# itsdfish/DifferentialEvolutionMCMC.jl

Measured on AMD Instinct MI355X. Metric: particle-updates/sec (proposal+loglike+accept) at D=32, N=1e5, higher is better.
Workload: dtype f64; 1 GPU; cfg3: MvNormal full-Sigma D=32, N=100000 obs, n_groups=256x1, Np=256, sampler defaults, schedule=two_colour, loglike=direct; particles_per_gpu=65536, parallelism=groups sharded x1, one all-gather per migration

## Files before the change

differentialevolutionmcmc.jl_amd/csrc/demc_hip.cpp:

```cpp
#include "../../include/demc.h"
#include "../../include/demc_summary.h"
#include "../../include/demc_quantile.h"

#include <hip/hip_runtime.h>
#include <hip/hip_ext.h>
#include <hip/hiprtc.h>
#include <rccl/rccl.h>

#include <algorithm>
#include <cmath>
#include <cstdio>
#include <cstdlib>
#include <cstring>
#include <exception>
#include <new>
#include <string>
#include <vector>

#define DEMC_K1_EXTERN
#include "demc_kernels.hpp"
#define DEMC_LONGROW_EXTERN
#include "demc_longrow.hpp"
#define DEMC_FROZEN_EXTERN
#include "demc_frozen.hpp"
// ... 315 lines not shown
}

#define DEMC_USER_KPARAMS                                                   \
    struct UserKParams {                                                    \
        int n_groups, Np, D, a_lo, n_act, n_chunks, nhyper, with_prior;     \
        long long N, P;                                                     \
        const double* prop;                                                 \
        double* partial;                                                    \
        const double* data;                                                 \
        const double* hyper;                                                \
        const long long* dims;                                              \
        const int* glist;                                                   \
        int ndims, pad;                                                     \
    };
DEMC_USER_KPARAMS
#define DEMC_STR_(...) #__VA_ARGS__
#define DEMC_STR(...) DEMC_STR_(__VA_ARGS__)
const char* kUserStruct = R"SRC(
#ifndef INFINITY
#define INFINITY __builtin_huge_val()
#endif
#ifndef NAN
#define NAN __builtin_nan("")
#endif
)SRC" DEMC_STR(DEMC_USER_KPARAMS) "\n";
const char* kUserPrologue = R"SRC(
__device__ double demc_user_obs(const double* theta, int D, const double* data, long long N, long long i,
                                const double* hyper, int nhyper);
)SRC";
const char* kUserRowPrologue = R"SRC(
__device__ double demc_user_loglike_row(const double* theta, int D, const double* data, const long long* dims, int ndims,
                                        const double* hyper, int nhyper, int lane, int n_lanes);
#ifdef DEMC_USER_HAS_PRIOR
__device__ double demc_user_prior_row(const double* theta, int D, const double* hyper, int nhyper, int lane, int n_lanes);
#endif
)SRC";
const char* kUserRowKernel = R"SRC(
extern "C" __global__ __launch_bounds__(256) void k_user_row(UserKParams p) {
    __shared__ double s_part[4];
    const int q = blockIdx.x;
    const int g = q / p.n_act;
    const size_t slot = (size_t)(p.glist ? p.glist[g] : g) * p.Np + p.a_lo + (q - g * p.n_act);
    const double* th = p.prop + slot * p.D;
    double acc = demc_user_loglike_row(th, p.D, p.data, p.dims, p.ndims, p.hyper, p.nhyper, (int)threadIdx.x, 256);
#ifdef DEMC_USER_HAS_PRIOR
    if (p.with_prior) acc += demc_user_prior_row(th, p.D, p.hyper, p.nhyper, (int)threadIdx.x, 256);
#endif
    for (int o = 32; o > 0; o >>= 1) acc += __shfl_xor(acc, o);
    if ((threadIdx.x & 63) == 0) s_part[threadIdx.x >> 6] = acc;
    __syncthreads();
    if (threadIdx.x == 0) p.partial[slot] = (s_part[0] + s_part[1]) + (s_part[2] + s_part[3]);
}
)SRC";
const char* kUserKernel = R"SRC(
extern "C" __global__ __launch_bounds__(256) void k_user_loglike(UserKParams p) {
    const int q = blockIdx.x * 256 + threadIdx.x;
    const int chunk = blockIdx.y;
    if (q >= p.n_groups * p.n_act) return;
    const int g = q / p.n_act;
    const size_t slot = (size_t)(p.glist ? p.glist[g] : g) * p.Np + p.a_lo + (q - g * p.n_act);
    const double* th = p.prop + slot * p.D;
    const long long per = (p.N + p.n_chunks - 1) / p.n_chunks;
    const long long i0 = chunk * per, i1 = (i0 + per < p.N) ? i0 + per : p.N;
    double acc = 0.0;
    for (long long i = i0; i < i1; ++i) acc += demc_user_obs(th, p.D, p.data, p.N, i, p.hyper, p.nhyper);
    p.partial[(size_t)chunk * p.P + slot] = acc;
}
)SRC";

int chunks_filling_rounds(long long blocks, long long cap, double resident_wgs) {
    long long best = 1;
    double best_fill = 0.0;
    for (long long nc = 1; nc <= cap; ++nc) {
        const double wgs = (double)blocks * (double)nc;
        const double fill = wgs / (std::ceil(wgs / resident_wgs) * resident_wgs);
        if (fill > best_fill + 1e-9 || (fill > best_fill - 1e-9 && wgs <= 4.0 * resident_wgs)) { best = nc; best_fill = fill; }
    }
    return (int)best;
}

int clock_buffer(demc_handle* h, size_t wgs, unsigned long long** out) {
    *out = nullptr;
    if (!h->timing) return DEMC_OK;
    if (wgs > h->clk_cap) {
        if (h->clk_dev) { HIPCHK(hipStreamSynchronize(h->stream)); hipFree(h->clk_dev); h->clk_dev = nullptr; h->clk_cap = 0; }
        ALLOC(h->clk_dev, 3 * wgs);
        h->clk_cap = wgs;
    }
    HIPCHK(hipMemsetAsync(h->clk_dev, 0, 3 * wgs * sizeof(unsigned long long), h->stream));
    h->clk_n = wgs;
    *out = h->clk_dev;
    return DEMC_OK;
}

const char* kSimKernelSource =
#include "demc_simlike_src.inc"
    ;

int launch_sim_loglike(demc_handle* h, KParams& k, long long n_prop) {
    SimKParams s;
    std::memset(&s, 0, sizeof s);
    s.n_groups = k.n_groups; s.Np = k.Np; s.D = k.D; s.a_lo = k.a_lo; s.n_act = k.n_act; s.group_offset = k.group_offset;
    s.n_sim = h->sim_n; s.nhyper = h->user_nhyper > 0 ? h->user_nhyper - 1 : 0;
    s.n_obs = h->N; s.iter = k.iter; s.seed = k.seed; s.sweep = k.sweep; s.entity_base = h->sim_entity_base;
    s.bandwidth = h->sim_bw; s.n_pow = std::pow((double)h->sim_n, -0.2);
    s.prop = k.prop; s.partial = k.partial; s.obs = h->data; s.hyper = h->user_hyper ? h->user_hyper + 1 : nullptr;
    s.logtab = h->sim_logtab; s.glist = k.glist; s.k_max = h->sim_kmax;
    const size_t lds = h->sim_est == EST_KDE_CHOICE ? sim_choice_lds(h->sim_n) : (size_t)h->sim_n * sizeof(double);
    h->last.k2 = demc_handle::K2_SIM; h->last.k2_key = InstKey{{h->sim_kind, h->sim_est}};
    if (h->sim_kind == SIM_USER) {
        size_t sz = sizeof s;
        void* cfg[] = {HIP_LAUNCH_PARAM_BUFFER_POINTER, &s, HIP_LAUNCH_PARAM_BUFFER_SIZE, &sz, HIP_LAUNCH_PARAM_END};
        tick(h, 2, true, true);
        const hipError_t e = hipModuleLaunchKernel(h->user_kernel, (unsigned)n_prop, 1, 1, 256, 1, 1, 0, h->stream, nullptr, cfg);
        tick(h, 2, false, true);
        if (e != hipSuccess) return fail(h, DEMC_EHIP, std::string("hipModuleLaunchKernel: ") + hipGetErrorString(e));
        return DEMC_OK;
    }
    const Inst<SimFn>* e = nullptr;
    PICK(e, "k_sim_loglike", kSim, h->sim_kind, h->sim_est);
    tick(h, 2, true);
    LAUNCH_T(h, e->fn, dim3((unsigned)n_prop), dim3(256), lds, s);
    tick(h, 2, false);
    return DEMC_OK;
}

int launch_ode_loglike(demc_handle* h, KParams& k) {
    OdeKParams o;
    std::memset(&o, 0, sizeof o);
    o.n_groups = k.n_groups; o.Np = k.Np; o.D = k.D; o.a_lo = k.a_lo; o.n_act = k.n_act;
    o.T = (int)h->N; o.substeps = h->ode_substeps;
    std::memcpy(o.u0, h->ode_u0, sizeof o.u0);
    o.h = h->ode_h; o.h2 = 0.5 * h->ode_h; o.h6 = h->ode_h / 6.0;
    o.prop = k.prop; o.partial = k.partial; o.obs = h->data; o.glist = k.glist;
    const Inst<OdeFn>* e = nullptr;
    PICK(e, "k_ode_loglike", kOde, ODE_LV);
    h->last.k2 = demc_handle::K2_ODE; h->last.k2_key = e->key;
    const size_t lds = (size_t)h->N * 2 * sizeof(double);
    tick(h, 2, true);
    LAUNCH_T(h, e->fn, dim3((unsigned)k.n_groups, (unsigned)((k.n_act + 255) / 256)), dim3(256), lds, o);
    tick(h, 2, false);
    return DEMC_OK;
}

int launch_loglike(demc_handle* h, KParams& k) {
    const long long n_prop = (long long)k.n_groups * k.n_act;
    if (n_prop == 0) return DEMC_OK;
    switch (h->family) {
        case FAM_MVN_FULL:
        case FAM_MVN_ISO: {
            const bool suff = h->c.loglike_mode == DEMC_LOGLIKE_SUFFSTAT;
            k.n_partials = 1;
            if (k.direct) {
                const long long blocks = (n_prop + 255) / 256;
                long long cap = h->N / 64;
                if (cap > h->partial_cap) cap = h->partial_cap;
                if (cap < 1) cap = 1;
                const Inst<ChunkFn>* e = nullptr;
                PICK(e, "k_direct_mvn", kDirect, h->dp_direct);
                if (int rc = wgs_per_cu(h, (const void*)e->fn, &h->direct_wgs_per_cu)) return rc;
                const int n_chunks = chunks_filling_rounds(blocks, cap, (double)h->direct_wgs_per_cu * h->n_cus);
                h->last.k2 = demc_handle::K2_DIRECT_MVN; h->last.k2_key = e->key;
                unsigned long long* clk = nullptr;
                if (int rc = clock_buffer(h, (size_t)blocks * (size_t)n_chunks, &clk)) return rc;
                tick(h, 2, true);
                LAUNCH_T(h, e->fn, dim3((unsigned)blocks, (unsigned)n_chunks), dim3(256), 0, k, n_chunks, clk);
                tick(h, 2, false);
                k.n_partials = n_chunks;
            } else if (!suff) {
                const Inst<CrossFn>* e = nullptr;
                PICK(e, "k_cross_mfma", kCross, h->ks_t <= 1 ? 1 : h->ks_t <= 2 ? 2 : h->ks_t <= 4 ? 4 : h->ks_t <= 8 ? 8 : 16, 4);
                h->last.k2 = demc_handle::K2_CROSS_MFMA; h->last.k2_key = e->key;
                tick(h, 2, true);
                const long long n_ptiles = (n_prop + 255) / 256;
                int n_chunks = 8;
                while (n_ptiles * n_chunks < 1024 && n_chunks * 2 <= 32 && h->n_tiles / (n_chunks * 2) >= 16) n_chunks *= 2;
                if (h->n_tiles < n_chunks) n_chunks = (int)(h->n_tiles > 0 ? h->n_tiles : 1);
                const int n_kpass = h->n_kpass;
                if (n_chunks * n_kpass > h->partial_cap) n_chunks = h->partial_cap / n_kpass;
                if (n_chunks < 1) return fail(h, DEMC_EINVAL, "data dimension too large for the partial-sum workspace");
                const int grid2 = (int)(n_ptiles * n_chunks);
                for (int kp = 0; kp < n_kpass; ++kp) {
                    const int k0 = kp * 4 * h->ks_t, part0 = kp * n_chunks;
                    LAUNCH_T(h, e->fn, dim3(grid2), dim3(256), 0, k, h->Ypad, h->dpad, k0, h->Xf, h->n_tiles, n_chunks, part0);
                }
                tick(h, 2, false);
                k.n_partials = n_chunks * n_kpass;
            }
        } break;
        case FAM_GAUSSIAN:
        case FAM_BINOMIAL:
        case FAM_LBA:
        case FAM_LNR:
        case FAM_RASTRIGIN: {
            long long cap = h->N / 32;
            if (cap > h->partial_cap) cap = h->partial_cap;
            if (cap < 1 || h->family == FAM_RASTRIGIN) cap = 1;
            if (int rc = wgs_per_cu(h, (const void*)k_obs_loglike, &h->obs_wgs_per_cu)) return rc;
            int n_chunks = chunks_filling_rounds((n_prop + 255) / 256, cap, (double)h->obs_wgs_per_cu * h->n_cus);
            if (h->family == FAM_LBA) {
                const Inst<ChunkFn>*e = nullptr, *e3 = nullptr;
                PICK(e, "k_lba_wave", kLbaWave, h->n_acc == 3 ? 3 : h->n_acc == 2 ? 2 : 0);
                PICK(e3, "k_lba_wave", kLbaWave, 3);
                if (int rc = wgs_per_cu(h, (const void*)e3->fn, &h->lba_wave_wgs_per_cu)) return rc;
                long long capw = h->N / 1024;
                if (capw > h->partial_cap) capw = h->partial_cap;
                if (capw < 1) capw = 1;
                int nc = chunks_filling_rounds((n_prop + 3) / 4, capw, (double)h->lba_wave_wgs_per_cu * h->n_cus);
                h->last.k2 = demc_handle::K2_LBA_WAVE;
                unsigned long long* clk = nullptr;
                if (int rc = clock_buffer(h, (size_t)((n_prop + 3) / 4) * (size_t)nc, &clk)) return rc;
                tick(h, 2, true);
                LAUNCH_T(h, e->fn, dim3((unsigned)((n_prop + 3) / 4), (unsigned)nc), dim3(256), 0, k, nc, clk);
                tick(h, 2, false);
                k.n_partials = nc;
                break;
            }
            h->last.k2 = demc_handle::K2_OBS;
            tick(h, 2, true);
            LAUNCH_T(h, k_obs_loglike, dim3((unsigned)((n_prop + 255) / 256), (unsigned)n_chunks), dim3(256), 0,
                               k, n_chunks);
            tick(h, 2, false);
            k.n_partials = n_chunks;
        } break;
        case FAM_USER: {
            long long want = (262144 + n_prop - 1) / n_prop;
            long long cap = h->N / 32;
            if (cap < 1) cap = 1;
            if (want > cap) want = cap;
            if (want > h->partial_cap) want = h->partial_cap;
            if (h->user_row) want = 1;
            UserKParams u;
            u.n_groups = k.n_groups; u.Np = k.Np; u.D = k.D; u.a_lo = k.a_lo; u.n_act = k.n_act; u.n_chunks = (int)want;
            u.nhyper = h->user_nhyper; u.with_prior = h->c.fitness_kind == DEMC_FITNESS_POSTERIOR ? 1 : 0;
            u.N = h->N; u.P = h->P; u.prop = k.prop; u.partial = k.partial;
            u.data = h->data; u.hyper = h->user_hyper; u.dims = h->user_dims; u.glist = k.glist; u.ndims = h->user_ndims; u.pad = 0;
            size_t sz = sizeof u;
            void* cfg[] = {HIP_LAUNCH_PARAM_BUFFER_POINTER, &u, HIP_LAUNCH_PARAM_BUFFER_SIZE, &sz, HIP_LAUNCH_PARAM_END};
            h->last.k2 = h->user_row ? demc_handle::K2_USER_ROW : demc_handle::K2_USER;
            tick(h, 2, true, true);
            hipError_t e = h->user_row
                ? hipModuleLaunchKernel(h->user_kernel, (unsigned)n_prop, 1, 1, 256, 1, 1, 0, h->stream, nullptr, cfg)
                : hipModuleLaunchKernel(h->user_kernel, (unsigned)((n_prop + 255) / 256), (unsigned)want, 1, 256, 1, 1, 0,
                                        h->stream, nullptr, cfg);
            tick(h, 2, false, true);
            if (e != hipSuccess) return fail(h, DEMC_EHIP, std::string("hipModuleLaunchKernel: ") + hipGetErrorString(e));
            k.n_partials = (int)want;
        } break;
        case FAM_SIM: {
            if (int rc = launch_sim_loglike(h, k, n_prop)) return rc;
            k.n_partials = 1;
        } break;
        case FAM_ODE_LV: {
            if (int rc = launch_ode_loglike(h, k)) return rc;
            k.n_partials = 1;
        } break;
        case FAM_HIER_BINOMIAL:
        case FAM_HIER_GAUSSIAN: {
            h->last.k2 = demc_handle::K2_HIER;
            tick(h, 2, true);
            LAUNCH_T(h, k_hier_loglike, dim3((unsigned)n_prop), dim3(256), 0, k);
            tick(h, 2, false);
            k.n_partials = 1;
        } break;
        default:
            return fail(h, DEMC_EUNSUPPORTED, "model family not set or not registered");
    }
    return DEMC_OK;
}

bool is_mvn(int fam) { return fam == FAM_MVN_FULL || fam == FAM_MVN_ISO; }

void set_tail_flags(demc_handle* h, KParams& k) {
    const demc_config& c = h->c;
    const bool suff = c.loglike_mode == DEMC_LOGLIKE_SUFFSTAT;
    k.fuse_prep = is_mvn(h->family) ? 1 : 0;
    k.prep_mfma = (h->family == FAM_MVN_FULL && k.lpp >= 4 && k.lpp <= 16 && h->d <= 32) ? 1 : 0;
    k.sx = (k.fuse_prep && suff) ? h->sx : nullptr;
    k.Ainv = (h->family == FAM_MVN_FULL) ? h->Ainv : nullptr;
    const long long obs_work = (h->family == FAM_HIER_GAUSSIAN) ? h->N * (h->d > 0 ? h->d : 1) : h->N;
    const bool cheap_obs = ((h->family == FAM_GAUSSIAN || h->family == FAM_BINOMIAL || h->family == FAM_RASTRIGIN) &&
                            h->N / k.lpp <= 512) ||
                           (h->hier_scr && obs_work / k.lpp <= 4096);
    const bool hist_private = c.schedule == DEMC_SCHED_SYNCHRONOUS && c.partner_kind == DEMC_PARTNER_HISTORY && k.mode == MODE_STEP &&
                              !(c.proposal_kind == 0 && k.iter <= c.burnin);
    const bool phase_private = c.schedule == DEMC_SCHED_TWO_COLOUR || c.schedule == DEMC_SCHED_SEQUENTIAL || k.mode == MODE_IDENT || hist_private;
    h->tf_cheap_obs = cheap_obs;
    k.fuse_obs = (cheap_obs && phase_private && c.fuse != 1) ? 1 : 0;
    k.fuse_accept = (((k.fuse_prep && suff) || k.fuse_obs) && c.fuse != 1 && phase_private) ? 1 : 0;
    k.write_prop = (!k.fuse_accept || k.trace) ? 1 : 0;
}
int lean_level(const demc_handle* h, const KParams& k) {
    const demc_config& c = h->c;
    const bool base = k.mode == MODE_STEP && c.proposal_kind == 0 && c.partner_kind == DEMC_PARTNER_CURRENT && c.update_kind == 0 &&
                      c.fitness_kind == 0 && c.kappa == 1.0 && !k.trace && !h->rp_active;
    return !base ? 0 : (c.theta_snooker == 0.0 && c.n_blocks == 0) ? 1 : 2;
}
bool is_plain(const demc_handle* h, const KParams& k) { return lean_level(h, k) == 1; }
int lean_hist(const demc_handle* h, const KParams& k) {
    const demc_config& c = h->c;
    const bool base = k.mode == MODE_STEP && c.proposal_kind == 0 && c.partner_kind == DEMC_PARTNER_HISTORY && c.update_kind == 0 &&
                      c.fitness_kind == 0 && c.kappa == 1.0 && !k.trace && !h->rp_active;
    return !base ? 0 : (c.theta_snooker == 0.0 && c.n_blocks == 0) ? 1 : 2;
}
int tail_of(const KParams& k) { return k.prep_mfma ? TAIL_PREP_MFMA : k.fuse_prep ? TAIL_PREP : k.fuse_obs ? TAIL_OBS : TAIL_NONE; }

int launch_phase(demc_handle* h, KParams k) {
    const long long n_prop = (long long)k.n_groups * k.n_act;
    if (n_prop == 0) return DEMC_OK;
    const demc_config& c = h->c;
    set_tail_flags(h, k);
    const int wg = k.lpp > 256 ? 512 : 256;
// ... 2233 lines not shown
```

differentialevolutionmcmc.jl_amd/csrc/demc_instances.hpp:

```cpp
#pragma once
#include <cstddef>
#include <string>

namespace demc {

constexpr int kMaxKey = 7;
struct InstKey { int v[kMaxKey]; };
constexpr bool same_key(const InstKey& a, const InstKey& b) {
    for (int i = 0; i < kMaxKey; ++i)
        if (a.v[i] != b.v[i]) return false;
    return true;
}

template <typename Fn>
struct Inst {
    Fn fn;
    InstKey key;
    std::string (*name)(const InstKey&);
};

template <typename I, size_t N>
constexpr const I* find_inst(const I (&tab)[N], const InstKey& key) {
    for (const I& e : tab)
        if (same_key(e.key, key)) return &e;
    return nullptr;
}
template <typename I, size_t N>
constexpr bool unique_keys(const I (&tab)[N]) {
    for (size_t i = 0; i < N; ++i)
        for (size_t j = i + 1; j < N; ++j)
            if (same_key(tab[i].key, tab[j].key)) return false;
    return true;
}

inline std::string int_list(const InstKey& k, int n) {
    std::string s;
    for (int i = 0; i < n; ++i) s += (i ? "," : "") + std::to_string(k.v[i]);
    return s;
}
inline const char* tf(int v) { return v == 0 ? "false" : v == 1 ? "true" : "2"; }
inline std::string name_propose(const InstKey& k) {
    static const char* const tails[4] = {"TAIL_NONE", "TAIL_PREP", "TAIL_PREP_MFMA", "TAIL_OBS"};
    return "k_propose<" + std::to_string(k.v[0]) + "," + tf(k.v[1]) + "," + tails[k.v[2] & 3] + "," + tf(k.v[3]) + "," + tf(k.v[4]) +
           (k.v[5] ? ",true>" : ">");
}
inline std::string name_res_mvn(const InstKey& k) {
    return "k_res_mvn<" + std::to_string(k.v[0]) + "," + tf(k.v[1]) + "," + std::to_string(k.v[2]) +
           (k.v[3] ? "," + std::to_string(k.v[3]) : "") + (k.v[5] ? ",iso" : "") + (k.v[6] ? ",direct" : "") + ">";
}
inline std::string name_frozen(const InstKey& k) { return "k_frozen_sweep<" + std::to_string(k.v[0]) + (k.v[3] ? ",big>" : ">"); }
inline std::string name_longrow(const InstKey& k) { return "k_longrow<" + int_list(k, 1) + ">"; }
inline std::string name_res_obs(const InstKey& k) { return "k_res_obs<" + int_list(k, 1) + ">"; }
inline std::string name_cross(const InstKey& k) { return "k_cross_mfma<" + int_list(k, 2) + ">"; }
inline std::string name_direct(const InstKey& k) { return "k_direct_mvn<" + int_list(k, 1) + ">"; }
inline std::string name_lba_wave(const InstKey&) { return "k_lba_wave"; }
inline std::string name_sim(const InstKey& k) {
    return std::string("k_sim_loglike<") + (k.v[1] == EST_KDE ? "kde" : k.v[1] == EST_FREQ ? "frequency" : "kde_choice") + "," +
           (k.v[0] == SIM_NORMAL ? "normal" : k.v[0] == SIM_BINOMIAL ? "binomial" : k.v[0] == SIM_LNR ? "lnr" : "user") + ">";
}
inline std::string name_ode(const InstKey& k) { return std::string("k_ode_loglike<") + (k.v[0] == ODE_LV ? "lv" : "?") + ">"; }

using K1Fn = void (*)(KParams);
using K1Inst = Inst<K1Fn>;
using ChunkFn = void (*)(KParams, int, unsigned long long*);
using CrossFn = void (*)(KParams, const double*, int, int, const double*, int, int, int);
using SimFn = void (*)(SimKParams);
using OdeFn = void (*)(OdeKParams);
#define DEMC_ENTRY(KERNEL, NAME, ...) {KERNEL<__VA_ARGS__>, {{__VA_ARGS__}}, NAME},
#define DEMC_E_PROPOSE(...) DEMC_ENTRY(k_propose, name_propose, __VA_ARGS__)
#define DEMC_E_RES_MVN(...) DEMC_ENTRY(k_res_mvn, name_res_mvn, __VA_ARGS__)
#define DEMC_E_FROZEN(...) DEMC_ENTRY(k_frozen_sweep, name_frozen, __VA_ARGS__)
#define DEMC_E_LONGROW(...) DEMC_ENTRY(k_longrow, name_longrow, __VA_ARGS__)
#define DEMC_E_RES_OBS(...) DEMC_ENTRY(k_res_obs, name_res_obs, __VA_ARGS__)
#define DEMC_E_DIRECT(...) DEMC_ENTRY(k_direct_mvn, name_direct, __VA_ARGS__)
#define DEMC_E_CROSS(...) DEMC_ENTRY(k_cross_mfma, name_cross, __VA_ARGS__)
#define DEMC_E_LBA_WAVE(...) DEMC_ENTRY(k_lba_wave, name_lba_wave, __VA_ARGS__)
#define DEMC_E_SIM(...) DEMC_ENTRY(k_sim_loglike, name_sim, __VA_ARGS__)
#define DEMC_E_SIM_CHOICE(SIM) {k_sim_choice<SIM>, {{SIM, EST_KDE_CHOICE}}, name_sim},
#define DEMC_E_ODE(...) DEMC_ENTRY(k_ode_loglike, name_ode, __VA_ARGS__)
constexpr K1Inst kPropose[] = {DEMC_K1_PHASE_INSTANCES(DEMC_E_PROPOSE) DEMC_K1_RES_INSTANCES(DEMC_E_PROPOSE) DEMC_K1_STREAM_INSTANCES(DEMC_E_PROPOSE)};
constexpr K1Inst kResMvn[] = {DEMC_RESMVN_INSTANCES(DEMC_E_RES_MVN) DEMC_RESMVN_INSTANCES_DIR(DEMC_E_RES_MVN)};
constexpr K1Inst kFrozen[] = {DEMC_FROZEN_INSTANCES(DEMC_E_FROZEN)};
constexpr K1Inst kLongrow[] = {DEMC_LONGROW_INSTANCES(DEMC_E_LONGROW)};
constexpr K1Inst kResObs[] = {DEMC_RESOBS_INSTANCES(DEMC_E_RES_OBS)};
constexpr Inst<ChunkFn> kDirect[] = {DEMC_DIRECT_INSTANCES(DEMC_E_DIRECT)};
constexpr Inst<CrossFn> kCross[] = {DEMC_CROSS_INSTANCES(DEMC_E_CROSS)};
constexpr Inst<ChunkFn> kLbaWave[] = {DEMC_LBA_WAVE_INSTANCES(DEMC_E_LBA_WAVE)};
constexpr Inst<SimFn> kSim[] = {DEMC_SIM_INSTANCES(DEMC_E_SIM) DEMC_SIM_CHOICE_INSTANCES(DEMC_E_SIM_CHOICE)};
constexpr Inst<OdeFn> kOde[] = {DEMC_ODE_INSTANCES(DEMC_E_ODE)};
static_assert(unique_keys(kPropose) && unique_keys(kResMvn) && unique_keys(kFrozen) && unique_keys(kLongrow) && unique_keys(kResObs) &&
                  unique_keys(kCross) && unique_keys(kDirect) && unique_keys(kLbaWave) && unique_keys(kSim) && unique_keys(kOde),
              "an instance list names the same template arguments twice");

}
```

differentialevolutionmcmc.jl_amd/csrc/demc_kernels.hpp:

```cpp
#pragma once
#include <type_traits>
#include "demc_device.hpp"

namespace demc {

enum Family : int {
    FAM_GAUSSIAN = 0, FAM_MVN_ISO = 1, FAM_MVN_FULL = 2, FAM_BINOMIAL = 3, FAM_HIER_BINOMIAL = 4,
    FAM_HIER_GAUSSIAN = 5, FAM_LBA = 6, FAM_LNR = 7, FAM_RASTRIGIN = 8, FAM_USER = 100
};
enum Mode : int { MODE_STEP = 0, MODE_IDENT = 1 };

struct DimTab {
    double lo, hi;
    double a, b;
    double c;
    int kind, ref;
};

struct DimSeg {
    int start, pad;
    DimTab t;
    double pad2;
};
constexpr int kMaxDimSeg = 16;
// ... 1629 lines not shown
        }
        DEMC_STAMP(20);
    }
    if (RES) __syncthreads();
    DEMC_STAMP(10);
    }
}

#define DEMC_K1_PHASE_INSTANCES(X) \
    X(256, false, TAIL_NONE, false, 0, false) X(256, false, TAIL_PREP, false, 0, false) \
    X(256, false, TAIL_PREP_MFMA, false, 0, false) X(256, false, TAIL_OBS, false, 0, false) \
    X(256, true, TAIL_NONE, false, 0, false) X(256, true, TAIL_PREP, false, 0, false) \
    X(256, true, TAIL_PREP_MFMA, false, 0, false) X(256, true, TAIL_OBS, false, 0, false) \
    X(256, true, TAIL_NONE, false, 1, false) X(256, true, TAIL_PREP, false, 1, false) \
    X(256, true, TAIL_PREP_MFMA, false, 1, false) X(256, true, TAIL_OBS, false, 1, false) \
    X(512, false, TAIL_NONE, false, 0, false) X(512, false, TAIL_PREP, false, 0, false) \
    X(512, false, TAIL_PREP_MFMA, false, 0, false) X(512, false, TAIL_OBS, false, 0, false) \
    X(256, true, TAIL_NONE, false, 2, false) X(256, true, TAIL_PREP, false, 2, false) \
    X(256, true, TAIL_PREP_MFMA, false, 2, false) X(256, true, TAIL_OBS, false, 2, false) \
    X(256, false, TAIL_NONE, false, 1, false) X(256, false, TAIL_PREP, false, 1, false) \
    X(256, false, TAIL_PREP_MFMA, false, 1, false) X(256, false, TAIL_OBS, false, 1, false) \
    X(256, false, TAIL_NONE, false, 2, false) X(256, false, TAIL_PREP, false, 2, false) \
    X(256, false, TAIL_PREP_MFMA, false, 2, false) X(256, false, TAIL_OBS, false, 2, false)
#define DEMC_K1_RES_INSTANCES(X) \
    X(256, true, TAIL_NONE, true, 0, false) X(256, true, TAIL_PREP, true, 0, false) \
    X(256, true, TAIL_PREP_MFMA, true, 0, false) X(256, true, TAIL_OBS, true, 0, false) \
    X(512, true, TAIL_NONE, true, 0, false) X(512, true, TAIL_PREP, true, 0, false) \
    X(512, true, TAIL_PREP_MFMA, true, 0, false) X(512, true, TAIL_OBS, true, 0, false) \
    X(256, true, TAIL_NONE, true, 1, false) X(256, true, TAIL_PREP, true, 1, false) \
    X(256, true, TAIL_PREP_MFMA, true, 1, false) X(256, true, TAIL_OBS, true, 1, false) \
    X(512, true, TAIL_NONE, true, 1, false) X(512, true, TAIL_PREP, true, 1, false) \
    X(512, true, TAIL_PREP_MFMA, true, 1, false) X(512, true, TAIL_OBS, true, 1, false) \
    X(256, true, TAIL_NONE, true, 2, false) X(256, true, TAIL_PREP, true, 2, false) \
    X(256, true, TAIL_PREP_MFMA, true, 2, false) X(256, true, TAIL_OBS, true, 2, false) \
    X(512, true, TAIL_NONE, true, 2, false) X(512, true, TAIL_PREP, true, 2, false) \
    X(512, true, TAIL_PREP_MFMA, true, 2, false) X(512, true, TAIL_OBS, true, 2, false)
#define DEMC_K1_STREAM_INSTANCES(X) \
    X(256, true, TAIL_PREP, true, 0, true) X(256, true, TAIL_PREP_MFMA, true, 0, true) \
    X(256, true, TAIL_PREP, true, 1, true) X(256, true, TAIL_PREP_MFMA, true, 1, true) \
    X(256, true, TAIL_PREP, true, 2, true) X(256, true, TAIL_PREP_MFMA, true, 2, true) \
    X(512, true, TAIL_PREP, true, 0, true) X(512, true, TAIL_PREP_MFMA, true, 0, true) \
    X(512, true, TAIL_PREP, true, 1, true) X(512, true, TAIL_PREP_MFMA, true, 1, true) \
    X(512, true, TAIL_PREP, true, 2, true) X(512, true, TAIL_PREP_MFMA, true, 2, true)
#ifdef DEMC_K1_EXTERN
#define DEMC_X_(...) extern template __global__ void k_propose<__VA_ARGS__>(KParams);
DEMC_K1_PHASE_INSTANCES(DEMC_X_)
DEMC_K1_RES_INSTANCES(DEMC_X_)
DEMC_K1_STREAM_INSTANCES(DEMC_X_)
#undef DEMC_X_
#endif

template <int KS, int MT>
__global__ __launch_bounds__(256, 2) void k_cross_mfma(KParams p, const double* __restrict__ Ypad, int dpad, int k0,
                                                       const double* __restrict__ Xf, int n_tiles, int n_chunks,
                                                       int part0) {
    const int lane = threadIdx.x & 63, wave = threadIdx.x >> 6;
    const int chunk = blockIdx.x % n_chunks;
    const int ptile = blockIdx.x / n_chunks;
    const int n_prop = p.n_groups * p.n_act;
    const int q0 = (ptile * 4 + wave) * (MT * 16);
    const int ksx = dpad >> 2;

    double a[MT][KS];
#pragma unroll
    for (int mt = 0; mt < MT; ++mt) {
        const int q = q0 + mt * 16 + (lane & 15);
        const bool ok = q < n_prop;
        const size_t slot = ok ? (size_t)slot_of(p, q) : 0;
        const double* yrow = Ypad + slot * dpad + k0 + (lane >> 4);
#pragma unroll
        for (int ks = 0; ks < KS; ++ks) {
            const double v = yrow[4 * ks];
            a[mt][ks] = ok ? v : 0.0;
        }
    }
    d4 acc[MT];
#pragma unroll
    for (int mt = 0; mt < MT; ++mt) acc[mt] = (d4){0.0, 0.0, 0.0, 0.0};

    const int per = (n_tiles + n_chunks - 1) / n_chunks;
    const int t0 = chunk * per, t1 = (t0 + per < n_tiles) ? t0 + per : n_tiles;
    const size_t tstride = (size_t)ksx * 64;
    const double* xb = Xf + (size_t)(k0 >> 2) * 64 + lane;
    double b0[KS], b1[KS];
    {
        const double* x = xb + (size_t)(t0 < t1 ? t0 : n_tiles) * tstride;
#pragma unroll
        for (int ks = 0; ks < KS; ++ks) b0[ks] = x[ks * 64];
    }
    for (int t = t0; t < t1; t += 2) {
        {
            const double* x = xb + (size_t)(t + 1 < t1 ? t + 1 : n_tiles) * tstride;
#pragma unroll
            for (int ks = 0; ks < KS; ++ks) b1[ks] = x[ks * 64];
        }
#pragma unroll
        for (int ks = 0; ks < KS; ++ks)
#pragma unroll
            for (int mt = 0; mt < MT; ++mt)
                acc[mt] = __builtin_amdgcn_mfma_f64_16x16x4f64(a[mt][ks], b0[ks], acc[mt], 0, 0, 0);
        {
            const double* x = xb + (size_t)(t + 2 < t1 ? t + 2 : n_tiles) * tstride;
#pragma unroll
            for (int ks = 0; ks < KS; ++ks) b0[ks] = x[ks * 64];
        }
#pragma unroll
        for (int ks = 0; ks < KS; ++ks)
#pragma unroll
            for (int mt = 0; mt < MT; ++mt)
                acc[mt] = __builtin_amdgcn_mfma_f64_16x16x4f64(a[mt][ks], b1[ks], acc[mt], 0, 0, 0);
    }
#pragma unroll
    for (int mt = 0; mt < MT; ++mt)
#pragma unroll
        for (int r = 0; r < 4; ++r) {
            double v = acc[mt][r];
            v += __shfl_xor(v, 1);
            v += __shfl_xor(v, 2);
            v += __shfl_xor(v, 4);
            v += __shfl_xor(v, 8);
            const int q = q0 + mt * 16 + (lane >> 4) + 4 * r;
            if ((lane & 15) == 0 && q < n_prop) p.partial[(size_t)(part0 + chunk) * p.P + slot_of(p, q)] = v;
        }
}
#define DEMC_CROSS_INSTANCES(X) X(1, 4) X(2, 4) X(4, 4) X(8, 4) X(16, 4)

template <int DP>
__device__ __forceinline__ void direct_mvn_rows(const KParams& p, int pblock, int chunk, int n_chunks) {
    const int q = pblock * 256 + threadIdx.x;
    const bool ok = q < p.n_groups * p.n_act;
    const size_t slot = ok ? (size_t)slot_of(p, q) : 0;
    double m[DP];
    const double* mrow = p.Ypad + slot * p.dpad;
#pragma unroll
    for (int k = 0; k < DP; ++k) m[k] = (ok && k < p.d) ? mrow[k] : 0.0;
    const long long per = (p.N + n_chunks - 1) / n_chunks;
    const long long i0 = chunk * per, i1 = (i0 + per < p.N) ? i0 + per : p.N;
    double acc[4] = {0.0, 0.0, 0.0, 0.0};
    const double* z = p.data + i0 * DP;
    for (long long i = i0; i < i1; ++i, z += DP) {
#pragma unroll
        for (int k = 0; k < DP; k += 4) {
#pragma unroll
            for (int e = 0; e < 4; ++e) {
                const double r = z[k + e] - m[k + e];
                acc[e] = fma(r, r, acc[e]);
            }
        }
    }
    if (ok) p.partial[(size_t)chunk * p.P + slot] = (acc[0] + acc[1]) + (acc[2] + acc[3]);
}

typedef int zs16 __attribute__((ext_vector_type(16)));
typedef double zd8 __attribute__((ext_vector_type(8)));
__device__ __forceinline__ void zslice_ask(zs16& lo, zs16& hi, const double* row) {
    asm volatile("s_load_dwordx16 %0, %2, 0x0\n\ts_load_dwordx16 %1, %2, 0x40" : "=&s"(lo), "=&s"(hi) : "s"(row) : "memory");
    __builtin_amdgcn_sched_barrier(0);
}
__device__ __forceinline__ void zslice_wait(zs16& lo, zs16& hi) {
    asm volatile("s_waitcnt lgkmcnt(0)" : "+s"(lo), "+s"(hi));
    __builtin_amdgcn_sched_barrier(0);
}
__device__ __forceinline__ void zslice_fma(const zs16& lo, const zs16& hi, const double (&m0)[16], const double (&m1)[16],
                                           double (&a0)[2], double (&a1)[2]) {
    const zd8 zl = __builtin_bit_cast(zd8, lo), zh = __builtin_bit_cast(zd8, hi);
#pragma unroll
    for (int k = 0; k < 16; ++k) {
        const double z = k < 8 ? zl[k & 7] : zh[k & 7];
        const double r0 = z - m0[k], r1 = z - m1[k];
        a0[k & 1] = fma(r0, r0, a0[k & 1]);
        a1[k & 1] = fma(r1, r1, a1[k & 1]);
    }
}
__device__ __forceinline__ void direct_mvn_slices(const KParams& p, int pblock, int chunk, int n_chunks) {
    __shared__ double s_other[256];
    __shared__ int s_slot[256];
    constexpr int kNoSlot = -1;
    const int lane = threadIdx.x & 63, wave = __builtin_amdgcn_readfirstlane(threadIdx.x >> 6);
    const int s = wave >> 1, h = wave & 1;
    const int n_prop = p.n_groups * p.n_act;
    const int t0 = h * 128 + lane, t1 = t0 + 64;
    double m0[16], m1[16];
    {
        const bool ok0 = pblock * 256 + t0 < n_prop, ok1 = pblock * 256 + t1 < n_prop;
        const int slot0 = ok0 ? slot_of(p, pblock * 256 + t0) : 0, slot1 = ok1 ? slot_of(p, pblock * 256 + t1) : 0;
        if (s == 0) {
            s_slot[t0] = ok0 ? slot0 : kNoSlot;
            s_slot[t1] = ok1 ? slot1 : kNoSlot;
        }
        const double *mrow0 = p.Ypad + (size_t)slot0 * p.dpad + 16 * s, *mrow1 = p.Ypad + (size_t)slot1 * p.dpad + 16 * s;
#pragma unroll
        for (int k = 0; k < 16; ++k) {
            m0[k] = (ok0 && 16 * s + k < p.d) ? mrow0[k] : 0.0;
            m1[k] = (ok1 && 16 * s + k < p.d) ? mrow1[k] : 0.0;
        }
    }
    const long long per = (p.N + n_chunks - 1) / n_chunks;
    const long long i0 = chunk * per, i1 = (i0 + per < p.N) ? i0 + per : p.N;
    const int n = (int)(i1 - i0);
    double a0[2] = {0.0, 0.0}, a1[2] = {0.0, 0.0};
    if (n > 0) {
        const double* z = p.data + i0 * 32 + 16 * s;
        zs16 alo, ahi, blo, bhi;
        zslice_ask(alo, ahi, z);
        for (int left = n; left >= 2; left -= 2, z += 64) {
            zslice_wait(alo, ahi);
            zslice_ask(blo, bhi, z + 32);
            zslice_fma(alo, ahi, m0, m1, a0, a1);
            zslice_wait(blo, bhi);
            zslice_ask(alo, ahi, left > 2 ? z + 64 : z + 32);
            zslice_fma(blo, bhi, m0, m1, a0, a1);
        }
        zslice_wait(alo, ahi);
        if (n & 1) zslice_fma(alo, ahi, m0, m1, a0, a1);
    }
    const double sum0 = a0[0] + a0[1], sum1 = a1[0] + a1[1];
    if (s == 1) {
        s_other[t0] = sum0;
        s_other[t1] = sum1;
    }
    __syncthreads();
    if (s == 0) {
        double* part = p.partial + (size_t)chunk * p.P;
        const int slot0 = s_slot[t0], slot1 = s_slot[t1];
        if (slot0 != kNoSlot) part[slot0] = sum0 + s_other[t0];
        if (slot1 != kNoSlot) part[slot1] = sum1 + s_other[t1];
    }
}

template <int DP>
__global__ __launch_bounds__(256) void k_direct_mvn(KParams p, int n_chunks, unsigned long long* __restrict__ clk) {
    int pblock = blockIdx.x, chunk = blockIdx.y;
    if ((n_chunks & 7) == 0) {
        const unsigned lin = blockIdx.y * gridDim.x + blockIdx.x, xcd = lin & 7u, j = lin >> 3;
        chunk = (int)((j / gridDim.x) * 8u + xcd);
        pblock = (int)(j % gridDim.x);
    }
    if constexpr (DP == 32)
        direct_mvn_slices(p, pblock, chunk, n_chunks);
    else
        direct_mvn_rows<DP>(p, pblock, chunk, n_chunks);
    if (clk) {
        const unsigned long long t1 = __builtin_amdgcn_s_memtime(), r1 = __builtin_amdgcn_s_memrealtime();
        const unsigned xcc = __builtin_amdgcn_s_getreg(20 | (3 << 11)) & 15u;
        const unsigned hwid = __builtin_amdgcn_s_getreg(4 | (31 << 11));
        if (threadIdx.x == 0) {
            const size_t wg = (size_t)blockIdx.y * gridDim.x + blockIdx.x;
            clk[3 * wg] = t1;
            clk[3 * wg + 1] = r1;
            clk[3 * wg + 2] = (xcc << 8) | ((hwid >> 8) & 0xffu);
        }
    }
}
#define DEMC_DIRECT_INSTANCES(X) X(8) X(16) X(32) X(64)

#ifndef DEMC_DEVICE_HELPERS_ONLY
__global__ __launch_bounds__(256) void k_obs_loglike(KParams p, int n_chunks) {
    constexpr int kTabPhi = kPhiIntervals * kPhiRow, kTabErfcx = kLogPhiRows * kLogPhiRow;
    __shared__ double s_tab[kTabPhi > kTabErfcx ? kTabPhi : kTabErfcx];
    if (p.family == FAM_LBA) {
        for (int i = threadIdx.x; i < kTabPhi; i += 256) s_tab[i] = kPhiTable[i];
        __syncthreads();
    } else if (p.family == FAM_LNR) {
        for (int i = threadIdx.x; i < kTabErfcx; i += 256) s_tab[i] = kLogPhiTable[i];
        __syncthreads();
    }
    const int q = blockIdx.x * 256 + threadIdx.x;
    const int n_prop = p.n_groups * p.n_act;
    const int chunk = blockIdx.y;
    if (q >= n_prop) return;
    const size_t slot = (size_t)slot_of(p, q);
    const double* th = p.prop + slot * p.D;
    const long long per = (p.N + n_chunks - 1) / n_chunks;
    const long long i0 = chunk * per, i1 = (i0 + per < p.N) ? i0 + per : p.N;
    double acc;
    if (p.family == FAM_LBA)
        acc = p.n_acc == 3 ? lba_range_sum<3>(p, th, i0, i1, 1, s_tab)
              : p.n_acc == 2 ? lba_range_sum<2>(p, th, i0, i1, 1, s_tab) : lba_range_sum<0>(p, th, i0, i1, 1, s_tab);
    else if (p.family == FAM_LNR)
        acc = lnr_range_sum(p, th, i0, i1, 1, s_tab);
    else
        acc = obs_range_sum(p, th, i0, i1, 1);
    p.partial[(size_t)chunk * p.P + slot] = acc;
}
#endif

#ifndef DEMC_DEVICE_HELPERS_ONLY
template <int NA>
__global__ __launch_bounds__(256, 2) void k_lba_wave(KParams p, int n_chunks, unsigned long long* __restrict__ clk) {
    __shared__ double s_tab[kPhiIntervals * kPhiRow];
    for (int i = threadIdx.x; i < kPhiIntervals * kPhiRow; i += 256) s_tab[i] = kPhiTable[i];
    __syncthreads();
    const int lane = threadIdx.x & 63, wave = __builtin_amdgcn_readfirstlane(threadIdx.x >> 6);
    const int q = blockIdx.x * 4 + wave;
    const int n_prop = p.n_groups * p.n_act;
    const int chunk = blockIdx.y;
    if (q >= n_prop) return;
    const size_t slot = (size_t)slot_of(p, q);
    const double* th = p.prop + slot * p.D;
    const int na = NA > 0 ? NA : p.n_acc;
    double nu[8], nuS[8];
#pragma unroll
    for (int a = 0; a < 8; ++a) {
        nu[a] = a < na ? th[a] : 0.0;
        nuS[a] = kPhiS * nu[a];
    }
    const double A = th[na], kk = th[na + 1], tau = th[na + 2], b = A + kk, inv_A = 1.0 / A;
    const double kS = kPhiS * kk, bS = kPhiS * b, inv_SA = inv_A * (1.0 / kPhiS);
    double pneg = 1.0;
#pragma unroll
    for (int a = 0; a < (NA > 0 ? NA : 8); ++a)
        if (a < na) {
            double qq, Ph;
            phiS_Phi_table(s_tab, -nuS[a], qq, Ph);
            pneg *= Ph;
        }
    const double inv_norm = 1.0 / (1.0 - pneg);
    constexpr long long kStep = 64LL * kLbaBatch;
    const long long n_steps = (p.N + kStep - 1) / kStep, per = (n_steps + n_chunks - 1) / n_chunks;
    const long long i0 = (long long)chunk * per * kStep, i1r = i0 + per * kStep, i1 = i1r < p.N ? i1r : p.N;
    double acc = 0.0;
    long long base = i0;
    for (; base + kStep <= i1; base += kStep) {
        double cc[kLbaBatch], rr[kLbaBatch];
#pragma unroll
        for (int j = 0; j < kLbaBatch; ++j) {
            cc[j] = p.data[base + 64LL * j + lane];
            rr[j] = p.data2[base + 64LL * j + lane];
        }
        double prod = 1.0;
#pragma unroll
        for (int j = 0; j < kLbaBatch; ++j)
            prod *= lba_trial<NA, double>(s_tab, na, nu, nuS, kS, bS, tau, inv_A, inv_SA, inv_norm, cc[j], rr[j]);
        if (__builtin_expect(!(prod < 1e300), 0)) {
            double s2 = 0.0;
#pragma unroll 1
            for (int j = 0; j < kLbaBatch; ++j)
                s2 += log(lba_trial<NA, double>(s_tab, na, nu, nuS, kS, bS, tau, inv_A, inv_SA, inv_norm, cc[j], rr[j]));
            acc += s2;
        } else
            acc += log(prod);
    }
#pragma unroll 1
    for (long long i = base + lane; i < i1; i += 64)
        acc += log(lba_trial<NA, double>(s_tab, na, nu, nuS, kS, bS, tau, inv_A, inv_SA, inv_norm, p.data[i], p.data2[i]));
    acc = subgroup_sum(acc, 64);
    if (lane == 0) p.partial[(size_t)chunk * p.P + slot] = acc;
    if (clk) {
        const unsigned long long t1 = __builtin_amdgcn_s_memtime(), r1 = __builtin_amdgcn_s_memrealtime();
        const unsigned xcc = __builtin_amdgcn_s_getreg(20 | (3 << 11)) & 15u, hwid = __builtin_amdgcn_s_getreg(4 | (31 << 11));
        if (threadIdx.x == 0) {
            const size_t wg = (size_t)blockIdx.y * gridDim.x + blockIdx.x;
            clk[3 * wg] = t1;
            clk[3 * wg + 1] = r1;
            clk[3 * wg + 2] = (xcc << 8) | ((hwid >> 8) & 0xffu);
        }
    }
}
#define DEMC_LBA_WAVE_INSTANCES(X) X(3) X(2) X(0)
#endif

#ifndef DEMC_DEVICE_HELPERS_ONLY
__global__ __launch_bounds__(256) void k_hier_loglike(KParams p) {
    __shared__ double s_part[4];
    const int tid = threadIdx.x, lane = tid & 63;
    const int q = blockIdx.x;
    const size_t slot = (size_t)slot_of(p, q);
    const double* th = p.prop + slot * p.D;
    const long long S = p.N;
    double acc = 0.0;
    if (p.family == FAM_HIER_BINOMIAL) {
        const double mu0 = th[0], n = p.c0;
        const double* lgc = p.data + S;
        for (long long s = tid; s < S; s += 256) {
            const double eta = mu0 + th[2 + s], k = p.data[s];
            acc += lgc[s] - n * softplus_fast(-eta) - (n - k) * eta;
        }
    } else {
        const double mu0 = th[0], sg = th[2 + S];
        const int n = p.d;
        const double lsg = log(sg), isg = 1.0 / sg;
        for (long long s = tid; s < S; s += 256) {
            const double mu = mu0 + th[2 + s];
            double l = 0.0;
            for (int i = 0; i < n; ++i) {
                const double z = (p.data[s * n + i] - mu) * isg;
                l += -(z * z + kLog2Pi) / 2.0 - lsg;
            }
            acc += l;
        }
    }
    for (int o = 32; o > 0; o >>= 1) acc += __shfl_xor(acc, o);
    if (lane == 0) s_part[tid >> 6] = acc;
    __syncthreads();
    if (tid == 0) p.partial[slot] = (s_part[0] + s_part[1]) + (s_part[2] + s_part[3]);
}
#endif

__device__ inline double sum_partials(const KParams& p, size_t slot, int sl, int lpp) {
    double s = 0.0;
    if (lpp > 64) {
        for (int c = 0; c < p.n_partials; ++c) s += p.partial[(size_t)c * p.P + slot];
        return s;
    }
    for (int c = sl; c < p.n_partials; c += lpp) s += p.partial[(size_t)c * p.P + slot];
    return subgroup_sum(s, lpp);
}
// ... 262 lines not shown
```

Measured before the change: 5.525 million particle-updates/s.

## Specialise direct MVN loglike by active width and add four-slice path for DP=64

Adds a width template parameter to the direct MVN kernel so scalar loads and FMAs cover only the active dimensions, rounded up to a step, instead of the full padded row. It also adds a four-wave slice variant for DP=64 with 128 proposals per workgroup and a multi-way shared-memory reduction. At D=32 the width equals 32, so the kernel does the same per-row work as before, now through the templated code path. The cost is more kernel instances and more complex load and reduction code.

```diff
diff --git a/differentialevolutionmcmc.jl_amd/csrc/demc_hip.cpp b/differentialevolutionmcmc.jl_amd/csrc/demc_hip.cpp
--- a/differentialevolutionmcmc.jl_amd/csrc/demc_hip.cpp
+++ b/differentialevolutionmcmc.jl_amd/csrc/demc_hip.cpp
@@ -491,12 +491,13 @@
             const bool suff = h->c.loglike_mode == DEMC_LOGLIKE_SUFFSTAT;
             k.n_partials = 1;
             if (k.direct) {
-                const long long blocks = (n_prop + 255) / 256;
+                const int width = direct_width(h->dp_direct, h->d);
+                const long long per_wg = direct_block_props(h->dp_direct, width), blocks = (n_prop + per_wg - 1) / per_wg;
                 long long cap = h->N / 64;
                 if (cap > h->partial_cap) cap = h->partial_cap;
                 if (cap < 1) cap = 1;
                 const Inst<ChunkFn>* e = nullptr;
-                PICK(e, "k_direct_mvn", kDirect, h->dp_direct);
+                PICK(e, "k_direct_mvn", kDirect, h->dp_direct, width);
                 if (int rc = wgs_per_cu(h, (const void*)e->fn, &h->direct_wgs_per_cu)) return rc;
                 const int n_chunks = chunks_filling_rounds(blocks, cap, (double)h->direct_wgs_per_cu * h->n_cus);
                 h->last.k2 = demc_handle::K2_DIRECT_MVN; h->last.k2_key = e->key;
diff --git a/differentialevolutionmcmc.jl_amd/csrc/demc_instances.hpp b/differentialevolutionmcmc.jl_amd/csrc/demc_instances.hpp
--- a/differentialevolutionmcmc.jl_amd/csrc/demc_instances.hpp
+++ b/differentialevolutionmcmc.jl_amd/csrc/demc_instances.hpp
@@ -52,7 +52,9 @@
 inline std::string name_longrow(const InstKey& k) { return "k_longrow<" + int_list(k, 1) + ">"; }
 inline std::string name_res_obs(const InstKey& k) { return "k_res_obs<" + int_list(k, 1) + ">"; }
 inline std::string name_cross(const InstKey& k) { return "k_cross_mfma<" + int_list(k, 2) + ">"; }
-inline std::string name_direct(const InstKey& k) { return "k_direct_mvn<" + int_list(k, 1) + ">"; }
+inline std::string name_direct(const InstKey& k) {
+    return "k_direct_mvn<" + int_list(k, 1) + ">" + (k.v[1] != k.v[0] ? "/w" + std::to_string(k.v[1]) : "");
+}
 inline std::string name_lba_wave(const InstKey&) { return "k_lba_wave"; }
 inline std::string name_sim(const InstKey& k) {
     return std::string("k_sim_loglike<") + (k.v[1] == EST_KDE ? "kde" : k.v[1] == EST_FREQ ? "frequency" : "kde_choice") + "," +
diff --git a/differentialevolutionmcmc.jl_amd/csrc/demc_kernels.hpp b/differentialevolutionmcmc.jl_amd/csrc/demc_kernels.hpp
--- a/differentialevolutionmcmc.jl_amd/csrc/demc_kernels.hpp
+++ b/differentialevolutionmcmc.jl_amd/csrc/demc_kernels.hpp
@@ -1805,47 +1805,100 @@
 }
 
 typedef int zs16 __attribute__((ext_vector_type(16)));
+typedef int zs8 __attribute__((ext_vector_type(8)));
+typedef int zs4 __attribute__((ext_vector_type(4)));
 typedef double zd8 __attribute__((ext_vector_type(8)));
-__device__ __forceinline__ void zslice_ask(zs16& lo, zs16& hi, const double* row) {
-    asm volatile("s_load_dwordx16 %0, %2, 0x0\n\ts_load_dwordx16 %1, %2, 0x40" : "=&s"(lo), "=&s"(hi) : "s"(row) : "memory");
+typedef double zd4 __attribute__((ext_vector_type(4)));
+typedef double zd2 __attribute__((ext_vector_type(2)));
+template <int SW>
+struct zslice {
+    static_assert(SW == 10 || SW == 12 || SW == 14 || SW == 16, "a slice is a 16-dword load and one or two shorter ones");
+    zs16 lo;
+    zs16 hi;
+    zs8 hi8;
+    zs4 hi4;
+};
+template <int SW>
+__device__ __forceinline__ void zslice_ask(zslice<SW>& t, const double* row) {
+    if constexpr (SW == 16)
+        asm volatile("s_load_dwordx16 %0, %2, 0x0\n\ts_load_dwordx16 %1, %2, 0x40" : "=&s"(t.lo), "=&s"(t.hi) : "s"(row) : "memory");
+    else if constexpr (SW == 14)
+        asm volatile("s_load_dwordx16 %0, %3, 0x0\n\ts_load_dwordx8 %1, %3, 0x40\n\ts_load_dwordx4 %2, %3, 0x60"
+                     : "=&s"(t.lo), "=&s"(t.hi8), "=&s"(t.hi4) : "s"(row) : "memory");
+    else if constexpr (SW == 12)
+        asm volatile("s_load_dwordx16 %0, %2, 0x0\n\ts_load_dwordx8 %1, %2, 0x40" : "=&s"(t.lo), "=&s"(t.hi8) : "s"(row) : "memory");
+    else
+        asm volatile("s_load_dwordx16 %0, %2, 0x0\n\ts_load_dwordx4 %1, %2, 0x40" : "=&s"(t.lo), "=&s"(t.hi4) : "s"(row) : "memory");
     __builtin_amdgcn_sched_barrier(0);
 }
-__device__ __forceinline__ void zslice_wait(zs16& lo, zs16& hi) {
-    asm volatile("s_waitcnt lgkmcnt(0)" : "+s"(lo), "+s"(hi));
+template <int SW>
+__device__ __forceinline__ void zslice_wait(zslice<SW>& t) {
+    if constexpr (SW == 16)
+        asm volatile("s_waitcnt lgkmcnt(0)" : "+s"(t.lo), "+s"(t.hi));
+    else if constexpr (SW == 14)
+        asm volatile("s_waitcnt lgkmcnt(0)" : "+s"(t.lo), "+s"(t.hi8), "+s"(t.hi4));
+    else if constexpr (SW == 12)
+        asm volatile("s_waitcnt lgkmcnt(0)" : "+s"(t.lo), "+s"(t.hi8));
+    else
+        asm volatile("s_waitcnt lgkmcnt(0)" : "+s"(t.lo), "+s"(t.hi4));
     __builtin_amdgcn_sched_barrier(0);
 }
-__device__ __forceinline__ void zslice_fma(const zs16& lo, const zs16& hi, const double (&m0)[16], const double (&m1)[16],
-                                           double (&a0)[2], double (&a1)[2]) {
-    const zd8 zl = __builtin_bit_cast(zd8, lo), zh = __builtin_bit_cast(zd8, hi);
-#pragma unroll
-    for (int k = 0; k < 16; ++k) {
-        const double z = k < 8 ? zl[k & 7] : zh[k & 7];
-        const double r0 = z - m0[k], r1 = z - m1[k];
+template <int SW>
+__device__ __forceinline__ void zslice_fma(const zslice<SW>& t, const double (&m0)[SW], const double (&m1)[SW], double (&a0)[2],
+                                           double (&a1)[2]) {
+    double z[SW];
+    {
+        const zd8 zl = __builtin_bit_cast(zd8, t.lo);
+#pragma unroll
+        for (int k = 0; k < 8; ++k) z[k] = zl[k];
+        if constexpr (SW == 16) {
+            const zd8 zh = __builtin_bit_cast(zd8, t.hi);
+#pragma unroll
+            for (int k = 0; k < 8; ++k) z[8 + k] = zh[k];
+        }
+        if constexpr (SW == 12 || SW == 14) {
+            const zd4 zh = __builtin_bit_cast(zd4, t.hi8);
+#pragma unroll
+            for (int k = 0; k < 4; ++k) z[8 + k] = zh[k];
+        }
+        if constexpr (SW == 10 || SW == 14) {
+            const zd2 zh = __builtin_bit_cast(zd2, t.hi4);
+            z[SW - 2] = zh[0];
+            z[SW - 1] = zh[1];
+        }
+    }
+#pragma unroll
+    for (int k = 0; k < SW; ++k) {
+        const double r0 = z[k] - m0[k], r1 = z[k] - m1[k];
         a0[k & 1] = fma(r0, r0, a0[k & 1]);
         a1[k & 1] = fma(r1, r1, a1[k & 1]);
     }
 }
+template <int DP, int NS, int SW>
 __device__ __forceinline__ void direct_mvn_slices(const KParams& p, int pblock, int chunk, int n_chunks) {
-    __shared__ double s_other[256];
-    __shared__ int s_slot[256];
+    static_assert((NS == 2 || NS == 4) && NS * SW <= DP, "two or four waves to a row share");
+    constexpr int H = 4 / NS;
+    constexpr int PB = 128 * H;
+    __shared__ double s_other[(NS - 1) * PB];
+    __shared__ int s_slot[PB];
     constexpr int kNoSlot = -1;
     const int lane = threadIdx.x & 63, wave = __builtin_amdgcn_readfirstlane(threadIdx.x >> 6);
-    const int s = wave >> 1, h = wave & 1;
+    const int s = wave / H, h = wave % H;
     const int n_prop = p.n_groups * p.n_act;
     const int t0 = h * 128 + lane, t1 = t0 + 64;
-    double m0[16], m1[16];
+    double m0[SW], m1[SW];
     {
-        const bool ok0 = pblock * 256 + t0 < n_prop, ok1 = pblock * 256 + t1 < n_prop;
-        const int slot0 = ok0 ? slot_of(p, pblock * 256 + t0) : 0, slot1 = ok1 ? slot_of(p, pblock * 256 + t1) : 0;
+        const bool ok0 = pblock * PB + t0 < n_prop, ok1 = pblock * PB + t1 < n_prop;
+        const int slot0 = ok0 ? slot_of(p, pblock * PB + t0) : 0, slot1 = ok1 ? slot_of(p, pblock * PB + t1) : 0;
         if (s == 0) {
             s_slot[t0] = ok0 ? slot0 : kNoSlot;
             s_slot[t1] = ok1 ? slot1 : kNoSlot;
         }
-        const double *mrow0 = p.Ypad + (size_t)slot0 * p.dpad + 16 * s, *mrow1 = p.Ypad + (size_t)slot1 * p.dpad + 16 * s;
-#pragma unroll
-        for (int k = 0; k < 16; ++k) {
-            m0[k] = (ok0 && 16 * s + k < p.d) ? mrow0[k] : 0.0;
-            m1[k] = (ok1 && 16 * s + k < p.d) ? mrow1[k] : 0.0;
+        const double *mrow0 = p.Ypad + (size_t)slot0 * p.dpad + SW * s, *mrow1 = p.Ypad + (size_t)slot1 * p.dpad + SW * s;
+#pragma unroll
+        for (int k = 0; k < SW; ++k) {
+            m0[k] = (ok0 && SW * s + k < p.d) ? mrow0[k] : 0.0;
+            m1[k] = (ok1 && SW * s + k < p.d) ? mrow1[k] : 0.0;
         }
     }
     const long long per = (p.N + n_chunks - 1) / n_chunks;
@@ -1853,35 +1906,43 @@
     const int n = (int)(i1 - i0);
     double a0[2] = {0.0, 0.0}, a1[2] = {0.0, 0.0};
     if (n > 0) {
-        const double* z = p.data + i0 * 32 + 16 * s;
-        zs16 alo, ahi, blo, bhi;
-        zslice_ask(alo, ahi, z);
-        for (int left = n; left >= 2; left -= 2, z += 64) {
-            zslice_wait(alo, ahi);
-            zslice_ask(blo, bhi, z + 32);
-            zslice_fma(alo, ahi, m0, m1, a0, a1);
-            zslice_wait(blo, bhi);
-            zslice_ask(alo, ahi, left > 2 ? z + 64 : z + 32);
-            zslice_fma(blo, bhi, m0, m1, a0, a1);
-        }
-        zslice_wait(alo, ahi);
-        if (n & 1) zslice_fma(alo, ahi, m0, m1, a0, a1);
+        const double* z = p.data + i0 * DP + SW * s;
+        zslice<SW> a, b;
+        zslice_ask(a, z);
+        for (int left = n; left >= 2; left -= 2, z += 2 * DP) {
+            zslice_wait(a);
+            zslice_ask(b, z + DP);
+            zslice_fma(a, m0, m1, a0, a1);
+            zslice_wait(b);
+            zslice_ask(a, left > 2 ? z + 2 * DP : z + DP);
+            zslice_fma(b, m0, m1, a0, a1);
+        }
+        zslice_wait(a);
+        if (n & 1) zslice_fma(a, m0, m1, a0, a1);
     }
     const double sum0 = a0[0] + a0[1], sum1 = a1[0] + a1[1];
-    if (s == 1) {
-        s_other[t0] = sum0;
-        s_other[t1] = sum1;
+    if (NS == 2 ? s == 1 : s != 0) {
+        s_other[(s - 1) * PB + t0] = sum0;
+        s_other[(s - 1) * PB + t1] = sum1;
     }
     __syncthreads();
     if (s == 0) {
         double* part = p.partial + (size_t)chunk * p.P;
         const int slot0 = s_slot[t0], slot1 = s_slot[t1];
-        if (slot0 != kNoSlot) part[slot0] = sum0 + s_other[t0];
-        if (slot1 != kNoSlot) part[slot1] = sum1 + s_other[t1];
-    }
-}
-
-template <int DP>
+        double r0 = sum0 + s_other[t0], r1 = sum1 + s_other[t1];
+#pragma unroll
+        for (int o = 1; o < NS - 1; ++o) {
+            r0 += s_other[o * PB + t0];
+            r1 += s_other[o * PB + t1];
+        }
+        if (slot0 != kNoSlot) part[slot0] = r0;
+        if (slot1 != kNoSlot) part[slot1] = r1;
+    }
+}
+
+constexpr int direct_slices(int DP, int ) { return DP == 32 ? 2 : DP == 64 ? 4 : 0; }
+constexpr int direct_block_props(int DP, int W) { return direct_slices(DP, W) == 4 ? 128 : 256; }
+template <int DP, int W>
 __global__ __launch_bounds__(256) void k_direct_mvn(KParams p, int n_chunks, unsigned long long* __restrict__ clk) {
     int pblock = blockIdx.x, chunk = blockIdx.y;
     if ((n_chunks & 7) == 0) {
@@ -1889,8 +1950,9 @@
         chunk = (int)((j / gridDim.x) * 8u + xcd);
         pblock = (int)(j % gridDim.x);
     }
-    if constexpr (DP == 32)
-        direct_mvn_slices(p, pblock, chunk, n_chunks);
+    constexpr int NS = direct_slices(DP, W);
+    if constexpr (NS != 0)
+        direct_mvn_slices<DP, NS, W / NS>(p, pblock, chunk, n_chunks);
     else
         direct_mvn_rows<DP>(p, pblock, chunk, n_chunks);
     if (clk) {
@@ -1905,7 +1967,13 @@
         }
     }
 }
-#define DEMC_DIRECT_INSTANCES(X) X(8) X(16) X(32) X(64)
+#define DEMC_DIRECT_INSTANCES(X) X(8, 8) X(16, 16) X(32, 20) X(32, 24) X(32, 28) X(32, 32) X(64, 40) X(64, 48) X(64, 56) X(64, 64)
+constexpr int direct_width(int DP, int d) {
+    const int step = DP == 32 ? 4 : DP == 64 ? 8 : 0;
+    if (step == 0) return DP;
+    const int w = (d + step - 1) / step * step;
+    return w < DP / 2 + step ? DP / 2 + step : w;
+}
 
 #ifndef DEMC_DEVICE_HELPERS_ONLY
 __global__ __launch_bounds__(256) void k_obs_loglike(KParams p, int n_chunks) {
```

New measurement: 5.540 million particle-updates/s (median of 3 runs). Within noise of the previous version (+0.3%).
